# goroda/c3sc

Hardware: AMD Instinct MI355X
Metric: Bellman-sweep nodes/sec (7D car rank-10) (higher is better)
Workload: dtype f64

## Files before the change

c3sc_amd/csrc/kernel_fiber_pair.hpp:

```cpp
#pragma once
#include <utility>

#include "fold_lds.hpp"

#ifndef FPP_CGD
#define FPP_CGD 3
#endif
#ifndef FPP_PIPE2
#define FPP_PIPE2 1
#endif
#ifndef FPP_CG
#define FPP_CG 1
#endif
#ifndef FPP_NV
#define FPP_NV 4
#endif

#ifndef FPP_DIRECT_MAXD
#define FPP_DIRECT_MAXD 3
#endif
#ifndef FPP_EDGE_TABLES
#define FPP_EDGE_TABLES 1
#endif

namespace c3sc {

constexpr int FPP_THREADS = 128;

template <class Model, int RP>
__host__ __device__ constexpr bool fpp_direct() { return Model::D <= FPP_DIRECT_MAXD && RP <= 8; }

template <class Model, int RP>
__host__ __device__ constexpr bool fpp_edge_tables() { return FPP_EDGE_TABLES && !fpp_direct<Model, RP>() && Model::D >= 4; }

template <int RP>
__device__ __forceinline__ void load_row16(const double *__restrict__ p, double (&r)[RP])
{
    typedef double v2d __attribute__((ext_vector_type(2)));
#pragma unroll
    for (int i = 0; i < RP / 2; i++) {
        const v2d v = *reinterpret_cast<const v2d *>(p + 2 * i);
        r[2 * i] = v.x;
        r[2 * i + 1] = v.y;
    }
}

template <int RP, int NW, int FIRST, int COUNT, bool ROWVEC>
__device__ inline void apply_core_and(const double *G, double (&W)[NW][RP], double (&E)[RP])
{
    constexpr int N1 = COUNT >= FPP_NV - 1 ? FPP_NV - 1 : COUNT;
    double tmp[N1 + 1][RP];
#pragma unroll
    for (int a = 0; a < RP; a++) tmp[0][a] = E[a];
#pragma unroll
    for (int s = 0; s < N1; s++)
#pragma unroll
        for (int a = 0; a < RP; a++) tmp[s + 1][a] = W[FIRST + s][a];
    if constexpr (ROWVEC) vecmat_lds<RP, N1 + 1>(G, tmp);
    else matvec_lds<RP, N1 + 1>(G, tmp);
#pragma unroll
    for (int a = 0; a < RP; a++) E[a] = tmp[0][a];
#pragma unroll
    for (int s = 0; s < N1; s++)
#pragma unroll
        for (int a = 0; a < RP; a++) W[FIRST + s][a] = tmp[s + 1][a];
    apply_core<RP, NW, FIRST + N1, COUNT - N1, ROWVEC, FPP_NV>(G, W);
}

__device__ inline void pair_barrier()
{
    asm volatile("s_waitcnt lgkmcnt(0)\n\ts_barrier" ::: "memory");
}

template <int H>
__device__ inline void stage_core_image(double *sK, const double *img, int n_doubles)
{
    typedef __attribute__((address_space(3))) char lds_char;
    typedef __attribute__((address_space(3))) void lds_void;
    typedef const __attribute__((address_space(1))) void glb_void;
    const int pieces = (n_doubles + 1) >> 1;
    const int lane = threadIdx.x & 63;
    for (int base = H * 64; base < pieces; base += FPP_THREADS) {
        const int b = max(min(base, pieces - 64), 0);
        const int p = min(b + lane, pieces - 1);
        __builtin_amdgcn_global_load_lds((glb_void *)(img + 2 * p), (lds_void *)((lds_char *)sK + 16 * b), 16, 0, 0);
    }
    asm volatile("s_waitcnt vmcnt(0)" ::: "memory");
}

template <int K>
__host__ __device__ constexpr int pair_owner(int m) { return m < K ? ((K - 1 - m) & 1) : ((m - K) & 1); }

template <class Model, int K>
struct PairPark {
    static constexpr int D = Model::D, NTAB = Model::NTAB;
    static constexpr unsigned UM = Model::UDEP_MASK, UC = Model::UCONST_MASK, ALL = (1u << D) - 1u;
    __host__ __device__ static constexpr bool has_deps()
    {
        if constexpr (requires { Model::HAS_DEPS; }) return Model::HAS_DEPS;
        else return false;
    }
    __host__ __device__ static constexpr unsigned dep(int m)
    {
        if constexpr (has_deps()) return Model::dep_mask(m);
        else return ALL;
    }
    __host__ __device__ static constexpr unsigned cost_dep()
    {
        if constexpr (has_deps()) return Model::COST_DEP;
        else return ALL;
    }
    __host__ __device__ static constexpr unsigned constd()
    {
        unsigned c = 0;
        if (has_deps())
            for (int m = 0; m < D; m++)
                if (!((UM >> m) & 1u) && !((dep(m) >> K) & 1u)) c |= 1u << m;
        return c;
    }
    __host__ __device__ static constexpr unsigned need()
    {
        unsigned n = cost_dep();
        for (int m = 0; m < D; m++) {
            const bool ctl = (UM >> m) & 1u, cst = (constd() >> m) & 1u;
            if ((!ctl && !cst) || (ctl && !((UC >> m) & 1u))) n |= dep(m);
        }
        return n & ALL;
    }
    __host__ __device__ static constexpr bool need_x(int m) { return m != K && ((need() >> m) & 1u); }
    __host__ __device__ static constexpr bool need_t(int t) { return Model::tab_dim(t) != K && ((need() >> Model::tab_dim(t)) & 1u); }
    __host__ __device__ static constexpr int row_x(int m)
    {
        int r = 0;
        for (int q = 0; q < m; q++) r += need_x(q);
        return r;
    }
    __host__ __device__ static constexpr int nx() { return row_x(D); }
    __host__ __device__ static constexpr int row_t(int t)
    {
        int r = nx();
        for (int q = 0; q < t; q++) r += need_t(q);
        return r;
    }
    __host__ __device__ static constexpr int nt() { return row_t(NTAB) - nx(); }
    __host__ __device__ static constexpr unsigned merged() { return constd() & ~(1u << K); }
    __host__ __device__ static constexpr unsigned rates() { return constd() & (1u << K); }
    __host__ __device__ static constexpr int row_pm(int m)
    {
        int r = nx() + nt();
        for (int q = 0; q < m; q++) r += 2 * ((rates() >> q) & 1u);
        return r;
    }
    __host__ __device__ static constexpr int row_q() { return row_pm(D); }
    __host__ __device__ static constexpr int rows() { return row_q() + (merged() != 0u); }
};

struct FoldPlan {
    int lfirst, rfirst;
    bool ledge, redge;
    int staged;
    int products;
};
template <class Model, int K, bool TAB = false>
struct PairMap {
    typedef PairPark<Model, K> PK;
    static constexpr int D = Model::D, NIT = D + 2, UL = D, UR = D + 1;
    __host__ __device__ static constexpr bool ltab() { return TAB && K >= 2; }
    __host__ __device__ static constexpr bool rtab() { return TAB && K <= D - 3; }
    __host__ __device__ static constexpr bool mg(int m) { return (PK::merged() >> m) & 1u; }
    __host__ __device__ static constexpr int first_l()
    {
        for (int m = 0; m < K; m++)
            if (mg(m)) return m;
        return -1;
    }
    __host__ __device__ static constexpr int first_r()
    {
        for (int m = D - 1; m > K; m--)
            if (mg(m)) return m;
        return -1;
    }
    __host__ __device__ static constexpr bool valid(int it)
    {
        return it == UL ? first_l() >= 0 : (it == UR ? first_r() >= 0 : (it != K && !mg(it)));
    }
    __host__ __device__ static constexpr int count(int it) { return !valid(it) ? 0 : (it < D ? 2 : 1); }
    __host__ __device__ static constexpr int nvl()
    {
        int c = count(UL);
        for (int m = 0; m < K; m++) c += count(m);
        return c;
    }
    __host__ __device__ static constexpr int nvr()
    {
        int c = count(UR);
        for (int m = K + 1; m < D; m++) c += count(m);
        return c;
    }
    __host__ __device__ static constexpr int nv() { return nvl() + nvr(); }
    __host__ __device__ static constexpr int gslot(int it)
    {
        if (it == UL) return 0;
        if (it == UR) return nvl();
        int c = it < K ? count(UL) : nvl() + count(UR);
        for (int m = it < K ? 0 : K + 1; m < it; m++) c += count(m);
        return c;
    }
    __host__ __device__ static constexpr int cost(int it)
    {
        if (!valid(it)) return 0;
        constexpr int lf = ltab() ? 2 : 1, rf = rtab() ? D - 3 : D - 2;
        if (it == UL) {
            int c = K - 1 - first_l() - (ltab() && first_l() == 0);
            for (int m = lf; m < K; m++) c += 2 * mg(m);
            return c;
        }
        if (it == UR) {
            int c = first_r() - K - 1 - (rtab() && first_r() == D - 1);
            for (int m = K + 1; m <= rf; m++) c += 2 * mg(m);
            return c;
        }
        if (it < K) return (ltab() && it <= 1) ? 2 * (K - 2) : (it > 0 ? 2 : 0) + 2 * (K - 1 - it);
        return (rtab() && it >= D - 2) ? 2 * (D - 3 - K) : (it < D - 1 ? 2 : 0) + 2 * (it - K - 1);
    }
    __host__ __device__ static constexpr FoldPlan plan()
    {
        FoldPlan p{ltab() ? 2 : 1, rtab() ? D - 3 : D - 2, K > 0 && !TAB, K < D - 1 && !TAB, 0, 0};
        const int ls = K - p.lfirst > 0 ? K - p.lfirst : 0, rs = p.rfirst - K > 0 ? p.rfirst - K : 0;
        p.staged = ls + rs + p.ledge + p.redge;
        p.products = ls + rs;
        for (int it = 0; it < NIT; it++) p.products += cost(it);
        return p;
    }
    __host__ __device__ static constexpr int owner(int it)
    {
        if (PK::merged() == 0u) return pair_owner<K>(it);
        int load[2] = {0, 0}, own[NIT] = {};
        bool done[NIT] = {};
        for (int n = 0; n < NIT; n++) {
            int best = -1;
            for (int q = 0; q < NIT; q++)
                if (valid(q) && !done[q] && (best < 0 || cost(q) > cost(best))) best = q;
            if (best < 0) break;
            const int h = load[1] < load[0] ? 1 : 0;
            own[best] = h;
            load[h] += cost(best);
            done[best] = true;
        }
        return own[it];
    }
    __host__ __device__ static constexpr int created(int m)
    {
        if (m == K) return -1;
        if (!mg(m)) return m;
        return m < K ? (m == first_l() ? UL : -1) : (m == first_r() ? UR : -1);
    }
    template <int H>
    __host__ __device__ static constexpr int left_before(int m)
    {
        int c = 0;
        for (int q = 0; q < m && q < K; q++)
            if (created(q) >= 0 && owner(created(q)) == H) c += count(created(q));
        return c;
    }
    template <int H>
    __host__ __device__ static constexpr int right_after(int m)
    {
        int c = 0;
        for (int q = D - 1; q > m && q > K; q--)
            if (created(q) >= 0 && owner(created(q)) == H) c += count(created(q));
        return c;
    }
    template <int H>
    __host__ __device__ static constexpr int lslot(int it)
    {
        if (it == UL) return left_before<H>(first_l());
        if (it == UR) return left_before<H>(K) + right_after<H>(first_r());
        return it < K ? left_before<H>(it) : left_before<H>(K) + right_after<H>(it);
    }
};

template <class Model, int K>
struct PairPre {
    static constexpr unsigned MASK = PairPark<Model, K>::merged(), RATES = PairPark<Model, K>::rates();
    const double *PX;
    int lane;
    double pvc;
    __device__ inline double q() const { return PX[PairPark<Model, K>::row_q() * 64 + lane]; }
    __device__ inline double pv() const { return pvc; }
    __device__ inline double pm(int m) const { return PX[PairPark<Model, K>::row_pm(m) * 64 + lane]; }
    __device__ inline double pp(int m) const { return PX[(PairPark<Model, K>::row_pm(m) + 1) * 64 + lane]; }
};

#define FPP_STAMP(slot)                                                   \
    if (C3SC_STAMPS_ON && (A.dbg & 128)) {                                \
        const unsigned long long now__ = clock64();                       \
        seg[slot] += now__ - tlast;                                       \
        tlast = now__;                                                    \
    }

template <class Model, int RP, int K, int H, bool FORCED>
__device__ __attribute__((always_inline)) inline void fiber_pair_body(const KArgs &A, const double *__restrict__ ro,
                                                                     const int32_t *__restrict__ idx, double *__restrict__ outv,
                                                                     int32_t *__restrict__ uidx, int32_t *__restrict__ absorbed,
                                                                     double *sK, unsigned &st)
{
    constexpr int D = Model::D;
    constexpr int S = 2 * D + 1;
    constexpr int RH = RP / 2;
    typedef PairPark<Model, K> PK;
    constexpr bool ET = fpp_edge_tables<Model, RP>();
    typedef PairMap<Model, K, ET> PM;
    constexpr FoldPlan PL = PM::plan();
    constexpr int NV = PM::nv();
    constexpr int NVL = PM::nvl();
    constexpr int NOL = PM::template left_before<H>(K);
    constexpr int NOR = PM::template right_after<H>(K);
    constexpr int NOWN = (NOL + NOR) > 0 ? (NOL + NOR) : 1;
    constexpr int NP = NV + 1;
    constexpr bool DIRECT = fpp_direct<Model, RP>();
    static_assert(RP % 2 == 0, "rank-split kernel needs an even padded rank");
    const int lane = threadIdx.x & 63;
    const int N = A.N;
    const long ntiles = (A.F + 63) / 64;
    unsigned long long seg[12] = {0, 0, 0, 0, 0, 0, 0, 0, 0, 0, 0, 0}, tlast = clock64();
    CandLds<Model> cr;
    NodeLds<Model, K> nr;
    {
        CandRegs<Model> cr0;
        cr0.load(A, ro);
        NodeRegs<Model, K> nr0;
        nr0.load(A, ro);
        double *tb = sK + A.tbl_off;
        cr.fill(tb, cr0, A.ncand);
        nr.fill(tb + CandLds<Model>::doubles(A.ncand), nr0, N);
        pair_barrier();
    }

    for (long tile = blockIdx.x; tile < ntiles; tile += gridDim.x) {
        FPP_STAMP(7)
        const long f_raw = tile * 64 + lane;
        const bool live = f_raw < A.F;
        const long f = live ? f_raw : A.F - 1;

        int fi[D], nbm[D], nbp[D];
        bool fiber_abs = false;
        double x[D];
#pragma unroll
        for (int m = 0; m < D; m++) {
            fi[m] = (m == K) ? 0 : idx[f * D + m];
            const bool face = fixed_neighbors(fi[m], A.ngrid[m], A.bctype[m], nbm[m], nbp[m]);
            if (m != K) fiber_abs = fiber_abs || face;
            x[m] = ro[A.xg_off[m] + fi[m]];
        }

        const unsigned obs_fixed = obstacle_mask_fixed<D>(A, ro, x, K);
        double tv[Model::NTAB > 0 ? Model::NTAB : 1];
        table_values<Model>(A, ro, fi, tv);

        double rpm[D], rpp[D];
#pragma unroll
        for (int m = 0; m < D; m++) { rpm[m] = 0.0; rpp[m] = 0.0; }
        if constexpr (PK::constd() != 0) {
            typename Model::Node nd0;
            Model::prep(A.prm, x, tv, nd0);
            double u0[Model::DU], cf0[Model::NCF > 0 ? Model::NCF : 1], b0[D], s0[D];
#pragma unroll
            for (int i = 0; i < Model::DU; i++) u0[i] = cr.get_u(i, 0);
            cf0[0] = 0.0;
#pragma unroll
            for (int i = 0; i < Model::NCF; i++) cf0[i] = cr.get_cf(i, 0);
            Model::drift(A.prm, nd0, x, u0, cf0, b0);
            Model::sigma(A.prm, x, u0, s0);
#pragma unroll
            for (int m = 0; m < D; m++)
                if ((PK::constd() >> m) & 1u) upwind_rates(A.t[2 * m], A.t[2 * m + 1], b0[m], s0[m], rpm[m], rpp[m]);
        }

        double L[RP], R[RP], W[NOWN][RP];
#pragma unroll
        for (int a = 0; a < RP; a++) { L[a] = (a == 0) ? 1.0 : 0.0; R[a] = (a == 0) ? 1.0 : 0.0; }

        FPP_STAMP(0)
        if (!(C3SC_STAMPS_ON && (A.dbg & 1))) {
        if constexpr (K > 0) {
            constexpr bool OWN0 = PM::ltab() && (PM::mg(0) ? PM::owner(PM::UL) == H : PM::owner(0) == H);
            constexpr bool OWN1 = PM::ltab() && (PM::mg(1) ? PM::owner(PM::UL) == H : PM::owner(1) == H);
            double t0m[OWN0 ? RP : 1], t0p[OWN0 ? RP : 1], t1m[OWN1 ? RP : 1], t1p[OWN1 ? RP : 1];
            if constexpr (PM::ltab()) {
                const double *T = ro + pair_tabL_off(A, RP);
                const int n1 = A.ngrid[1];
                load_row16<RP>(T + ((long)fi[0] * n1 + fi[1]) * RP, L);
                if constexpr (OWN0) {
                    load_row16<RP>(T + ((long)nbm[0] * n1 + fi[1]) * RP, t0m);
                    load_row16<RP>(T + ((long)nbp[0] * n1 + fi[1]) * RP, t0p);
                }
                if constexpr (OWN1) {
                    load_row16<RP>(T + ((long)fi[0] * n1 + nbm[1]) * RP, t1m);
                    load_row16<RP>(T + ((long)fi[0] * n1 + nbp[1]) * RP, t1p);
                }
                __builtin_amdgcn_sched_barrier(0);
            }
            auto left_combine = [&]() __attribute__((always_inline)) {
                if constexpr (OWN0) {
#pragma unroll
                    for (int b = 0; b < RP; b++) {
                        if constexpr (PM::mg(0)) W[0][b] = fma(rpp[0], t0p[b], rpm[0] * t0m[b]);
                        else { W[0][b] = t0m[b]; W[1][b] = t0p[b]; }
                    }
                }
                if constexpr (OWN1) {
                    constexpr int before = PM::template left_before<H>(1);
#pragma unroll
                    for (int b = 0; b < RP; b++) {
                        if constexpr (PM::mg(1)) {
                            constexpr int su = PM::template lslot<H>(PM::UL);
                            const double nw = fma(rpp[1], t1p[b], rpm[1] * t1m[b]);
                            W[su][b] = (1 == PM::first_l()) ? nw : W[su][b] + nw;
                        } else { W[before][b] = t1m[b]; W[before + 1][b] = t1p[b]; }
                    }
                }
            };
            if constexpr (PM::ltab() && K == PL.lfirst) left_combine();
            if constexpr (!PM::ltab()) {
                constexpr bool GLB = DIRECT || !PL.ledge;
                constexpr int str = GLB ? RP : fpl_lds_stride(RP);
                const double *src = sK;
                FPP_STAMP(1)
                if constexpr (GLB) src = ro + A.core_off[0];
                else {
                    pair_barrier();
                    stage_core_image<H>(sK, A.img_base + A.pair_img_off[0], A.ngrid[0] * str);
                    pair_barrier();
                }
                FPP_STAMP(7)
#pragma unroll
                for (int b = 0; b < RP; b++) {
                    L[b] = src[fi[0] * str + b];
                    if constexpr (PM::mg(0)) {
                        if constexpr (PM::owner(PM::UL) == H) W[0][b] = fma(rpp[0], src[nbp[0] * str + b], rpm[0] * src[nbm[0] * str + b]);
                    } else if constexpr (PM::owner(0) == H) {
                        W[0][b] = src[nbm[0] * str + b];
                        W[1][b] = src[nbp[0] * str + b];
                    }
                }
            }
            auto left_step = [&](auto mc) __attribute__((always_inline)) {
                constexpr int m = decltype(mc)::value;
                constexpr int str = DIRECT ? RP * RP : fpl_lds_stride(RP * RP);
                constexpr int before = PM::template left_before<H>(m);
                constexpr bool PAIR = !PM::mg(m) && PM::owner(m) == H, ACC = PM::mg(m) && PM::owner(PM::UL) == H;
                double nw[RP];
                const double *src = sK;
                FPP_STAMP(1)
                if constexpr (DIRECT) src = ro + A.core_off[m];
                else {
                    pair_barrier();
                    stage_core_image<H>(sK, A.img_base + A.pair_img_off[m], A.ngrid[m] * str);
                    pair_barrier();
                }
                if constexpr (PM::ltab() && m == PL.lfirst) left_combine();
                FPP_STAMP(7)
                const double *G = src + fi[m] * str;
                if constexpr (PAIR || ACC) {
                    double t0[1][RP], t1[1][RP];
#pragma unroll
                    for (int a = 0; a < RP; a++) { t0[0][a] = L[a]; t1[0][a] = L[a]; }
                    if constexpr (DIRECT) {
                        apply_glb<RP, 1, true>(src + nbm[m] * str, t0);
                        apply_glb<RP, 1, true>(src + nbp[m] * str, t1);
                    } else {
                        vecmat_lds<RP, 1>(src + nbm[m] * str, t0);
                        vecmat_lds<RP, 1>(src + nbp[m] * str, t1);
                    }
#pragma unroll
                    for (int a = 0; a < RP; a++) {
                        if constexpr (PAIR) { W[before][a] = t0[0][a]; W[before + 1][a] = t1[0][a]; }
                        else nw[a] = fma(rpp[m], t1[0][a], rpm[m] * t0[0][a]);
                    }
                }
                if constexpr (DIRECT) {
                    double tl[1][RP];
#pragma unroll
                    for (int a = 0; a < RP; a++) tl[0][a] = L[a];
                    apply_glb<RP, 1, true>(G, tl);
#pragma unroll
                    for (int a = 0; a < RP; a++) L[a] = tl[0][a];
                    apply_range_glb<RP, NOWN, 0, before, true>(G, W);
                } else
                    apply_core_and<RP, NOWN, 0, before, true>(G, W, L);
                if constexpr (ACC) {
                    constexpr int su = PM::template lslot<H>(PM::UL);
#pragma unroll
                    for (int a = 0; a < RP; a++) W[su][a] = (m == PM::first_l()) ? nw[a] : W[su][a] + nw[a];
                }
            };
            [&]<int... Ms>(std::integer_sequence<int, Ms...>) { (left_step(std::integral_constant<int, Ms + PL.lfirst>{}), ...); }
            (std::make_integer_sequence<int, (K > PL.lfirst ? K - PL.lfirst : 0)>{});
        }

        if constexpr (K < D - 1) {
            constexpr bool OWN0 = PM::rtab() && (PM::mg(D - 1) ? PM::owner(PM::UR) == H : PM::owner(D - 1) == H);
            constexpr bool OWN1 = PM::rtab() && (PM::mg(D - 2) ? PM::owner(PM::UR) == H : PM::owner(D - 2) == H);
            double t0m[OWN0 ? RP : 1], t0p[OWN0 ? RP : 1], t1m[OWN1 ? RP : 1], t1p[OWN1 ? RP : 1];
            if constexpr (PM::rtab()) {
                const double *T = ro + pair_tabR_off(A, RP);
                const int n1 = A.ngrid[D - 1];
                load_row16<RP>(T + ((long)fi[D - 2] * n1 + fi[D - 1]) * RP, R);
                if constexpr (OWN0) {
                    load_row16<RP>(T + ((long)fi[D - 2] * n1 + nbm[D - 1]) * RP, t0m);
                    load_row16<RP>(T + ((long)fi[D - 2] * n1 + nbp[D - 1]) * RP, t0p);
                }
                if constexpr (OWN1) {
                    load_row16<RP>(T + ((long)nbm[D - 2] * n1 + fi[D - 1]) * RP, t1m);
                    load_row16<RP>(T + ((long)nbp[D - 2] * n1 + fi[D - 1]) * RP, t1p);
                }
                __builtin_amdgcn_sched_barrier(0);
            }
            auto right_combine = [&]() __attribute__((always_inline)) {
                if constexpr (OWN0) {
#pragma unroll
                    for (int a = 0; a < RP; a++) {
                        if constexpr (PM::mg(D - 1)) W[NOL][a] = fma(rpp[D - 1], t0p[a], rpm[D - 1] * t0m[a]);
                        else { W[NOL][a] = t0m[a]; W[NOL + 1][a] = t0p[a]; }
                    }
                }
                if constexpr (OWN1) {
                    constexpr int after = PM::template right_after<H>(D - 2);
#pragma unroll
                    for (int a = 0; a < RP; a++) {
                        if constexpr (PM::mg(D - 2)) {
                            constexpr int su = PM::template lslot<H>(PM::UR);
                            const double nw = fma(rpp[D - 2], t1p[a], rpm[D - 2] * t1m[a]);
                            W[su][a] = (D - 2 == PM::first_r()) ? nw : W[su][a] + nw;
                        } else { W[NOL + after][a] = t1m[a]; W[NOL + after + 1][a] = t1p[a]; }
                    }
                }
            };
            if constexpr (PM::rtab() && K == PL.rfirst) right_combine();
            if constexpr (!PM::rtab()) {
                constexpr bool GLB = DIRECT || !PL.redge;
                constexpr int str = GLB ? RP : fpl_lds_stride(RP);
                const double *src = sK;
                FPP_STAMP(1)
                if constexpr (GLB) src = ro + A.core_off[D - 1];
                else {
                    pair_barrier();
                    stage_core_image<H>(sK, A.img_base + A.pair_img_off[D - 1], A.ngrid[D - 1] * str);
                    pair_barrier();
                }
                FPP_STAMP(7)
#pragma unroll
                for (int a = 0; a < RP; a++) {
                    R[a] = src[fi[D - 1] * str + a];
                    if constexpr (PM::mg(D - 1)) {
                        if constexpr (PM::owner(PM::UR) == H)
                            W[NOL][a] = fma(rpp[D - 1], src[nbp[D - 1] * str + a], rpm[D - 1] * src[nbm[D - 1] * str + a]);
                    } else if constexpr (PM::owner(D - 1) == H) {
                        W[NOL][a] = src[nbm[D - 1] * str + a];
                        W[NOL + 1][a] = src[nbp[D - 1] * str + a];
                    }
                }
            }
            auto right_step = [&](auto mc) __attribute__((always_inline)) {
                constexpr int m = decltype(mc)::value;
                constexpr int str = DIRECT ? RP * RP : fpl_lds_stride(RP * RP);
                constexpr int after = PM::template right_after<H>(m);
                constexpr bool PAIR = !PM::mg(m) && PM::owner(m) == H, ACC = PM::mg(m) && PM::owner(PM::UR) == H;
                double nw[RP];
                const double *src = sK;
                FPP_STAMP(1)
                if constexpr (DIRECT) src = ro + A.core_off[m];
                else {
                    pair_barrier();
                    stage_core_image<H>(sK, A.img_base + A.pair_img_off[m], A.ngrid[m] * str);
                    pair_barrier();
                }
                if constexpr (PM::rtab() && m == PL.rfirst) right_combine();
                FPP_STAMP(7)
                const double *G = src + fi[m] * str;
                if constexpr (PAIR || ACC) {
                    double t0[1][RP], t1[1][RP];
#pragma unroll
                    for (int a = 0; a < RP; a++) { t0[0][a] = R[a]; t1[0][a] = R[a]; }
                    if constexpr (DIRECT) {
                        apply_glb<RP, 1, false>(src + nbm[m] * str, t0);
                        apply_glb<RP, 1, false>(src + nbp[m] * str, t1);
                    } else {
                        matvec_lds<RP, 1>(src + nbm[m] * str, t0);
                        matvec_lds<RP, 1>(src + nbp[m] * str, t1);
                    }
#pragma unroll
                    for (int a = 0; a < RP; a++) {
                        if constexpr (PAIR) { W[NOL + after][a] = t0[0][a]; W[NOL + after + 1][a] = t1[0][a]; }
                        else nw[a] = fma(rpp[m], t1[0][a], rpm[m] * t0[0][a]);
                    }
                }
                if constexpr (DIRECT) {
                    double tr[1][RP];
#pragma unroll
                    for (int a = 0; a < RP; a++) tr[0][a] = R[a];
                    apply_glb<RP, 1, false>(G, tr);
#pragma unroll
                    for (int a = 0; a < RP; a++) R[a] = tr[0][a];
                    apply_range_glb<RP, NOWN, NOL, after, false>(G, W);
                } else
                    apply_core_and<RP, NOWN, NOL, after, false>(G, W, R);
                if constexpr (ACC) {
                    constexpr int su = PM::template lslot<H>(PM::UR);
#pragma unroll
                    for (int a = 0; a < RP; a++) W[su][a] = (m == PM::first_r()) ? nw[a] : W[su][a] + nw[a];
                }
            };
            [&]<int... Ms>(std::integer_sequence<int, Ms...>) { (right_step(std::integral_constant<int, PL.rfirst - Ms>{}), ...); }
            (std::make_integer_sequence<int, (PL.rfirst - K > 0 ? PL.rfirst - K : 0)>{});
        }

        }
        FPP_STAMP(1)
        double Wh[NV][RH];
        {
            double *X = sK;
            pair_barrier();
            auto put_get_own = [&](auto ic) __attribute__((always_inline)) {
                constexpr int it = decltype(ic)::value;
                if constexpr (PM::valid(it) && PM::owner(it) == H) {
                    constexpr int slot = PM::template lslot<H>(it);
#pragma unroll
                    for (int s = 0; s < PM::count(it); s++) {
                        const int g = PM::gslot(it) + s;
#pragma unroll
                        for (int i = 0; i < RH; i++) {
                            X[(g * RH + i) * 64 + lane] = W[slot + s][(1 - H) * RH + i];
                            Wh[g][i] = W[slot + s][H * RH + i];
                        }
                    }
                }
            };
            [&]<int... Ms>(std::integer_sequence<int, Ms...>) { (put_get_own(std::integral_constant<int, Ms>{}), ...); }
            (std::make_integer_sequence<int, PM::NIT>{});
            pair_barrier();
            auto get_other = [&](auto ic) __attribute__((always_inline)) {
                constexpr int it = decltype(ic)::value;
                if constexpr (PM::valid(it) && PM::owner(it) != H) {
#pragma unroll
                    for (int s = 0; s < PM::count(it); s++) {
                        const int g = PM::gslot(it) + s;
#pragma unroll
                        for (int i = 0; i < RH; i++) Wh[g][i] = X[(g * RH + i) * 64 + lane];
                    }
                }
            };
            [&]<int... Ms>(std::integer_sequence<int, Ms...>) { (get_other(std::integral_constant<int, Ms>{}), ...); }
            (std::make_integer_sequence<int, PM::NIT>{});
            pair_barrier();
        }
        double *sL = sK, *sR = sK + RP * 64;
        {
#pragma unroll
            for (int a = 0; a < RP; a++) {
                if constexpr (H == 0) sL[a * 64 + lane] = L[a];
                else sR[a * 64 + lane] = R[a];
            }
            if constexpr (H == 0) {
                static_assert(PK::rows() <= NP, "parking rows exceed the reserved block");
                double *PXw = sK + (2 * RP + 2 * (NP + 1) + NP) * 64;
#pragma unroll
                for (int m = 0; m < D; m++)
                    if (PK::need_x(m)) PXw[PK::row_x(m) * 64 + lane] = x[m];
#pragma unroll
                for (int t = 0; t < Model::NTAB; t++)
                    if (PK::need_t(t)) PXw[PK::row_t(t) * 64 + lane] = tv[t];
#pragma unroll
                for (int m = 0; m < D; m++)
                    if ((PK::rates() >> m) & 1u) {
                        PXw[PK::row_pm(m) * 64 + lane] = rpm[m];
                        PXw[(PK::row_pm(m) + 1) * 64 + lane] = rpp[m];
                    }
                if constexpr (PK::merged() != 0u) {
                    double qc = 0.0;
#pragma unroll
                    for (int m = 0; m < D; m++)
                        if (PM::mg(m)) { qc += rpm[m]; qc += rpp[m]; }
                    PXw[PK::row_q() * 64 + lane] = qc;
                }
            }
            pair_barrier();
        }
        FPP_STAMP(2)

        const int bck = A.bctype[K];
        const double *Gk = ro + A.core_off[K];
        auto partials = [&](int j, auto &&sink) __attribute__((always_inline)) -> double {
            double pv;
            if constexpr (K == 0) {
                double ah[RH];
#pragma unroll
                for (int i = 0; i < RH; i++) ah[i] = Gk[(size_t)j * RP + H * RH + i];
                double v = 0.0;
#pragma unroll
                for (int i = 0; i < RH; i++) v = fma(ah[i], sR[(H * RH + i) * 64 + lane], v);
                pv = v;
#pragma unroll
                for (int g = 0; g < NV; g++) sink(g, dot_reg<RH>(ah, Wh[g]));
            } else if constexpr (K == D - 1) {
                double ch[RH];
#pragma unroll
                for (int i = 0; i < RH; i++) ch[i] = Gk[(size_t)j * RP + H * RH + i];
                double v = 0.0;
#pragma unroll
                for (int i = 0; i < RH; i++) v = fma(sL[(H * RH + i) * 64 + lane], ch[i], v);
                pv = v;
#pragma unroll
                for (int g = 0; g < NV; g++) sink(g, dot_reg<RH>(Wh[g], ch));
            } else {
                const double *GC0 = Gk + (size_t)j * RP * RP;
                const double *GC = GC0 + (size_t)H * RH * RP;
                double ch[RH], ah[RH];
#pragma unroll
                for (int i = 0; i < RH; i++) { ch[i] = 0.0; ah[i] = 0.0; }
#pragma unroll
                for (int b = 0; b < RP; b++) {
                    const double rb = sR[b * 64 + lane];
#pragma unroll
                    for (int i = 0; i < RH; i++) ch[i] = fma(GC0[H * RH + i + b * RP], rb, ch[i]);
                }
#pragma unroll
                for (int a = 0; a < RP; a++) {
                    const double la = sL[a * 64 + lane];
#pragma unroll
                    for (int i = 0; i < RH; i++) ah[i] = fma(la, GC[a + i * RP], ah[i]);
                }
                double v = 0.0;
#pragma unroll
                for (int i = 0; i < RH; i++) v = fma(sL[(H * RH + i) * 64 + lane], ch[i], v);
                pv = v;
#pragma unroll
                for (int g = 0; g < NVL; g++) sink(g, dot_reg<RH>(Wh[g], ch));
#pragma unroll
                for (int g = NVL; g < NV; g++) sink(g, dot_reg<RH>(ah, Wh[g]));
            }
            sink(NV, pv);
            return pv;
        };
        auto to_lds = [&](double *dst) __attribute__((always_inline)) {
            return [dst, lane](int g, double v) __attribute__((always_inline)) { dst[g * 64 + lane] = v; };
        };
        auto ca_part = [&](int j, double (&ch)[RH], double (&ah)[RH], auto &&filler) __attribute__((always_inline)) {
            const double *GC0 = Gk + (size_t)j * RP * RP;
            const double *GC = GC0 + (size_t)H * RH * RP;
#pragma unroll
            for (int i = 0; i < RH; i++) { ch[i] = 0.0; ah[i] = 0.0; }
            constexpr int BH = (RP + 1) / 2;
            double vec[RP];
#pragma unroll
            for (int b = 0; b < RP; b++) vec[b] = sR[b * 64 + lane];
#pragma unroll
            for (int b0 = 0; b0 < RP; b0 += BH) {
                double g[BH][RH];
#pragma unroll
                for (int b = 0; b < BH; b++)
#pragma unroll
                    for (int i = 0; i < RH; i++) g[b][i] = (b0 + b < RP) ? GC0[H * RH + i + (b0 + b) * RP] : 0.0;
                __builtin_amdgcn_sched_barrier(0);
                filler(b0 / BH);
                __builtin_amdgcn_sched_barrier(0);
#pragma unroll
                for (int b = 0; b < BH; b++)
#pragma unroll
                    for (int i = 0; i < RH; i++) asm volatile("" : "+s"(g[b][i]));
#pragma unroll
                for (int b = 0; b < BH; b++) {
                    if (b0 + b < RP) {
                        const double rb = vec[b0 + b];
#pragma unroll
                        for (int i = 0; i < RH; i++) ch[i] = fma(g[b][i], rb, ch[i]);
                    }
                }
            }
#pragma unroll
            for (int a = 0; a < RP; a++) vec[a] = sL[a * 64 + lane];
#pragma unroll
            for (int a0 = 0; a0 < RP; a0 += BH) {
                double g[RH][BH];
#pragma unroll
                for (int i = 0; i < RH; i++)
#pragma unroll
                    for (int a = 0; a < BH; a++) g[i][a] = (a0 + a < RP) ? GC[a0 + a + i * RP] : 0.0;
                __builtin_amdgcn_sched_barrier(0);
                filler(2 + a0 / BH);
                __builtin_amdgcn_sched_barrier(0);
#pragma unroll
                for (int i = 0; i < RH; i++)
#pragma unroll
                    for (int a = 0; a < BH; a++) asm volatile("" : "+s"(g[i][a]));
#pragma unroll
                for (int a = 0; a < BH; a++) {
                    if (a0 + a < RP) {
                        const double la = vec[a0 + a];
#pragma unroll
                        for (int i = 0; i < RH; i++) ah[i] = fma(la, g[i][a], ah[i]);
                    }
                }
            }
        };
        auto dots_quarter = [&](int q, const double (&ch)[RH], const double (&ah)[RH], auto &&sink) __attribute__((always_inline)) {
#pragma unroll
            for (int g = 0; g < NV; g++)
                if (g * 4 / NV == q) sink(g, (g < NVL) ? dot_reg<RH>(Wh[g], ch) : dot_reg<RH>(ah, Wh[g]));
        };
        auto dots_part = [&](const double (&ch)[RH], const double (&ah)[RH], auto &&sink) __attribute__((always_inline)) -> double {
            double v = 0.0;
#pragma unroll
            for (int i = 0; i < RH; i++) v = fma(sL[(H * RH + i) * 64 + lane], ch[i], v);
#pragma unroll
            for (int g = 0; g < NVL; g++) sink(g, dot_reg<RH>(Wh[g], ch));
#pragma unroll
            for (int g = NVL; g < NV; g++) sink(g, dot_reg<RH>(ah, Wh[g]));
            sink(NV, v);
            return v;
        };
        double *B0 = sK + 2 * RP * 64;
        double *B1 = B0 + (NP + 1) * 64;
        double *B2 = B1 + (NP + 1) * 64;
        double *PX = B2 + NP * 64;

        auto finalize = [&](int jn, const double (&Vt)[NP], double vlo, double vhi) __attribute__((always_inline)) {
            double V[S];
#pragma unroll
            for (int m = 0; m < D; m++) {
                if (m == K) { V[2 * m] = vlo; V[2 * m + 1] = vhi; }
                else if (PM::mg(m)) { V[2 * m] = 0.0; V[2 * m + 1] = 0.0; }
                else { V[2 * m] = Vt[PM::gslot(m)]; V[2 * m + 1] = Vt[PM::gslot(m) + 1]; }
            }
            V[2 * D] = Vt[NV];
            double pvc = 0.0;
            if constexpr (PM::valid(PM::UL)) pvc += Vt[PM::gslot(PM::UL)];
            if constexpr (PM::valid(PM::UR)) pvc += Vt[PM::gslot(PM::UR)];
            double x[D], tv[Model::NTAB > 0 ? Model::NTAB : 1];
            tv[0] = 0.0;
#pragma unroll
            for (int m = 0; m < D; m++)
                x[m] = (m == K) ? nr.x_at(jn) : (PairPark<Model, K>::need_x(m) ? PX[PairPark<Model, K>::row_x(m) * 64 + lane] : 0.0);
#pragma unroll
            for (int t = 0; t < Model::NTAB; t++)
                tv[t] = (Model::tab_dim(t) == K) ? nr.tab_at(t, jn)
                                                 : (PairPark<Model, K>::need_t(t) ? PX[PairPark<Model, K>::row_t(t) * 64 + lane] : 0.0);
            int ab = (obs_fixed & nr.mask_at(jn)) ? -1 : 0;
            if (fiber_abs) ab = 1;
            int lo, hi;
            ab = vary_neighbors(jn, N, bck, ab, lo, hi, A.cends);
            int ui;
            FPP_STAMP(8)
            int fu = -1;
            if constexpr (FORCED) fu = A.forced[(size_t)f * N + jn];
            const PairPre<Model, K> pre{PX, lane, pvc};
            const double val = node_backup<Model, FPP_CG, FPP_CGD, CandLds<Model>, true, PairPre<Model, K>>(A, ro, x, tv, cr, V, ab, ui, st, FORCED, fu, pre);
            FPP_STAMP(9)
            outv[(size_t)f * N + jn] = val;
            if (uidx) uidx[(size_t)f * N + jn] = ui;
            if (absorbed) absorbed[(size_t)f * N + jn] = ab;
        };

        double vwrap = 0.0;
        if (bck == C3SC_PERIODIC) {
            const double pv = partials(N - 2, [](int, double) __attribute__((always_inline)) {});
            if constexpr (H == 0) B0[NP * 64 + lane] = pv;
            else B1[NP * 64 + lane] = pv;
            pair_barrier();
            vwrap = pv + (H == 0 ? B1[NP * 64 + lane] : B0[NP * 64 + lane]);
            pair_barrier();
        }
        double vone = 0.0;
        double v_m2 = 0.0, v_m1 = 0.0;
        double Vd[NP];
#pragma unroll
        for (int g = 0; g < NP; g++) Vd[g] = 0.0;

        const int T = N / 2 + 1;
        for (int t = 0; t < T; t++) {
            const int j0 = 2 * t, j1 = 2 * t + 1;
            const bool has0 = j0 < N, has1 = j1 < N;
            double pv0 = 0.0, pv1 = 0.0;
            double Pown[NP];
#pragma unroll
            for (int g = 0; g < NP; g++) Pown[g] = 0.0;
            auto own_sink = [&](int g, double v) __attribute__((always_inline)) { Pown[g] = v; };
            if constexpr (K > 0 && K < D - 1 && FPP_PIPE2) {
                if (has0 && has1) {
                    double chA[RH], ahA[RH], chB[RH], ahB[RH];
                    auto nofill = [](int) __attribute__((always_inline)) {};
                    auto value_of = [&](const double (&ch)[RH]) __attribute__((always_inline)) -> double {
                        double v = 0.0;
#pragma unroll
                        for (int i = 0; i < RH; i++) v = fma(sL[(H * RH + i) * 64 + lane], ch[i], v);
                        return v;
                    };
                    if constexpr (H == 0) {
                        auto sinkA = to_lds(B0);
                        ca_part(j1, chA, ahA, nofill);
                        ca_part(j0, chB, ahB, [&](int q) __attribute__((always_inline)) { dots_quarter(q, chA, ahA, sinkA); });
                        pv1 = value_of(chA);
                        sinkA(NV, pv1);
                        pv0 = dots_part(chB, ahB, own_sink);
                        B0[NP * 64 + lane] = pv0;
                    } else {
                        auto sinkA = to_lds(B1);
                        ca_part(j0, chA, ahA, nofill);
                        ca_part(j1, chB, ahB, [&](int q) __attribute__((always_inline)) { dots_quarter(q, chA, ahA, sinkA); });
                        pv0 = value_of(chA);
                        sinkA(NV, pv0);
                        pv1 = dots_part(chB, ahB, to_lds(B2));
                        B1[NP * 64 + lane] = pv1;
                    }
                } else if (has0) {
                    if constexpr (H == 0) { pv0 = partials(j0, own_sink); B0[NP * 64 + lane] = pv0; }
                    else pv0 = partials(j0, to_lds(B1));
                }
            } else if constexpr (H == 0) {
                if (has1) pv1 = partials(j1, to_lds(B0));
                if (has0) {
                    pv0 = partials(j0, own_sink);
                    B0[NP * 64 + lane] = pv0;
                }
            } else {
                if (has0) pv0 = partials(j0, to_lds(B1));
                if (has1) {
                    pv1 = partials(j1, to_lds(B2));
                    B1[NP * 64 + lane] = pv1;
                }
            }
            FPP_STAMP(3)
            pair_barrier();
            FPP_STAMP(4)
            double v0 = 0.0, v1 = 0.0;
            if constexpr (H == 0) {
                if (has1) v1 = pv1 + B1[NP * 64 + lane];
                if (has0) {
                    double P0[NP];
#pragma unroll
                    for (int g = 0; g < NP; g++) P0[g] = Pown[g] + B1[g * 64 + lane];
                    v0 = P0[NV];
                    double vlo, vhi;
                    dimk_values(j0, N, bck, v_m1, v0, v1, vwrap, (j0 == 0 ? v1 : vone), vlo, vhi);
                    finalize(j0, P0, vlo, vhi);
                }
            } else {
                if (has0) v0 = pv0 + B0[NP * 64 + lane];
                if (t >= 1) {
                    const int jn = j0 - 1;
                    double vlo, vhi;
                    dimk_values(jn, N, bck, v_m2, Vd[NV], v0, vwrap, (jn == 1 ? Vd[NV] : vone), vlo, vhi);
                    finalize(jn, Vd, vlo, vhi);
                }
                if (has1) {
#pragma unroll
                    for (int g = 0; g < NP; g++) Vd[g] = B0[g * 64 + lane] + B2[g * 64 + lane];
                    v1 = Vd[NV];
                }
            }
            if (t == 0) vone = v1;
            v_m2 = v0;
            v_m1 = v1;
            FPP_STAMP(5)
            pair_barrier();
            FPP_STAMP(6)
        }
    }
    if (C3SC_STAMPS_ON && (A.dbg & 128) && lane == 0) {
        const size_t w = ((size_t)blockIdx.x * 2 + H) * 12;
        if (w < 65536 * 8)
            for (int i = 0; i < 12; i++) A.dbgbuf[w + i] = seg[i];
    }
}

#ifndef FPP_WPS_LOW
#define FPP_WPS_LOW 4
#endif
#ifndef FPP_WPS_HIGH
#define FPP_WPS_HIGH 2
#endif
template <class Model, int RP>
__host__ __device__ constexpr int fpp_waves_per_simd() { return (fpp_direct<Model, RP>() && RP <= 6) ? FPP_WPS_LOW : (FPP_WPS_HIGH); }

template <class Model, int RP, int K, bool FORCED>
__global__ void __launch_bounds__(FPP_THREADS, (fpp_waves_per_simd<Model, RP>()))
    k_fiber_pair(const KArgs A, const double *__restrict__ ro, const int32_t *__restrict__ idx, double *__restrict__ outv,
                 int32_t *__restrict__ uidx, int32_t *__restrict__ absorbed)
{
    extern __shared__ double sKp[];
    unsigned st = 0;
    const int h = __builtin_amdgcn_readfirstlane(threadIdx.x >> 6);
    if (h == 0) fiber_pair_body<Model, RP, K, 0, FORCED>(A, ro, idx, outv, uidx, absorbed, sKp, st);
    else fiber_pair_body<Model, RP, K, 1, FORCED>(A, ro, idx, outv, uidx, absorbed, sKp, st);
    if (st) atomicOr(A.status, st);
}

}
```

c3sc_amd/csrc/launch_fpp.hpp:

```cpp
#pragma once
#include "kernel_fiber_pair.hpp"
#include "registry.hpp"

namespace c3sc {

template <class Model, int RP, int K, bool FORCED>
hipError_t launch_fpp_impl(const KArgs &A, const LaunchIO &io)
{
    constexpr int D = Model::D;
    constexpr int NV = PairMap<Model, K>::nv(), NP = NV + 1, RH = RP / 2;
    if (A.ncand > 64) return hipErrorNotSupported;
    size_t doubles = (size_t)NV * RH * 64;
    const size_t exch = (size_t)(2 * RP + (NP + 1) * 2 + 2 * NP) * 64;
    if (exch > doubles) doubles = exch;
    for (int m = 0; m < D; m++) {
        if (m == K || fpp_direct<Model, RP>()) continue;
        const int elems = (m == 0 || m == D - 1) ? RP : RP * RP;
        const size_t need = ((size_t)A.ngrid[m] * fpl_lds_stride(elems) + 1) & ~(size_t)1;
        if (need > doubles) doubles = need;
    }
    KArgs B = A;
    B.tbl_off = (int)doubles;
    doubles += (size_t)CandLds<Model>::doubles(A.ncand) + (size_t)NodeLds<Model, K>::doubles(A.N);
    const size_t shmem = doubles * sizeof(double);
    auto kern = k_fiber_pair<Model, RP, K, FORCED>;
    static LaunchCache cache;
    int blocks_per_cu = 1, num_cu = 256;
    hipError_t e = cache.prepare((const void *)kern, FPP_THREADS, shmem, blocks_per_cu, num_cu);
    if (e != hipSuccess) return e;
    const long ntiles = (A.F + 63) / 64;
    const long cap = (long)num_cu * blocks_per_cu;
    int grid = (int)(ntiles < cap ? ntiles : cap);
    if (ntiles >= 8 * cap && ntiles < 0x7fffffffL) grid = (int)ntiles;
    if (grid < 1) grid = 1;
    hipLaunchKernelGGL(kern, dim3(grid), dim3(FPP_THREADS), shmem, io.stream, B, io.ro, io.idx, io.out, io.uidx, io.absorbed);
    return hipGetLastError();
}

template <class Model, int RP, int K>
hipError_t launch_fpp(const KArgs &A, const LaunchIO &io)
{
    return A.forced ? launch_fpp_impl<Model, RP, K, true>(A, io) : launch_fpp_impl<Model, RP, K, false>(A, io);
}

#define C3SC_REG_FPP1(MODEL_ID, RP, K, ...)                                                                   \
    static Registrar C3SC_CAT(reg_fpp_, __COUNTER__)(KernelEntry{                                             \
        MODEL_ID, __VA_ARGS__::D, RP, 0, C3SC_VARIANT_FIBER_PAIR, 128, K, &launch_fpp<__VA_ARGS__, RP, K>, \
        "k_fiber_pair<" #__VA_ARGS__ "," #RP ",K=" #K ">"});

}
```

Before: 29.86 billion.

## Split fiber-pair node work by node parity instead of by rank half

Adds a node-split mode where each wave of the pair keeps full-rank W vectors (exchanged via LDS in two halves) and computes the complete stencil for alternating nodes, instead of each wave computing half-rank partials that are summed through LDS every node. This removes per-node partial-sum exchange and one barrier per step, at the cost of more VGPRs (full NV×RP registers) and duplicated stencil reads. It is gated by a VGPR budget and opts out for rank<10 and the 7D rank-10 K=4 case. LDS sizing is refactored into a helper with static asserts.

Result: faster. 31.40 billion (median of 6 runs) (+5.2%).

```diff
diff --git a/c3sc_amd/csrc/kernel_fiber_pair.hpp b/c3sc_amd/csrc/kernel_fiber_pair.hpp
--- a/c3sc_amd/csrc/kernel_fiber_pair.hpp
+++ b/c3sc_amd/csrc/kernel_fiber_pair.hpp
@@ -21,6 +21,13 @@
 #endif
 #ifndef FPP_EDGE_TABLES
 #define FPP_EDGE_TABLES 1
+#endif
+
+#ifndef FPP_NODE_SPLIT
+#define FPP_NODE_SPLIT 1
+#endif
+#ifndef FPP_NODE_SPLIT_VGPRS
+#define FPP_NODE_SPLIT_VGPRS 140
 #endif
 
 namespace c3sc {
@@ -279,6 +286,16 @@
         return it < K ? left_before<H>(it) : left_before<H>(K) + right_after<H>(it);
     }
 };
+
+__host__ __device__ constexpr bool fpp_node_split_optout(int d, int rp, int k) { return rp < 10 || (d == 7 && rp == 10 && k == 4); }
+template <class Model, int RP, int K>
+__host__ __device__ constexpr bool fpp_node_split()
+{
+    if constexpr (!FPP_NODE_SPLIT || fpp_direct<Model, RP>()) return false;
+    else
+        return PairPark<Model, K>::merged() != 0u && PairMap<Model, K>::nv() * RP * 2 <= FPP_NODE_SPLIT_VGPRS &&
+               !fpp_node_split_optout(Model::D, RP, K);
+}
 
 template <class Model, int K>
 struct PairPre {
@@ -618,8 +635,49 @@
 
         }
         FPP_STAMP(1)
-        double Wh[NV][RH];
-        {
+        constexpr bool NS = fpp_node_split<Model, RP, K>();
+        double Wh[NS ? 1 : NV][RH];
+        double Wf[NS ? NV : 1][RP];
+        if constexpr (NS) {
+            double *X = sK;
+            auto put_get_own = [&](auto ic, auto pc) __attribute__((always_inline)) {
+                constexpr int it = decltype(ic)::value, P = decltype(pc)::value;
+                if constexpr (PM::valid(it) && PM::owner(it) == H) {
+                    constexpr int slot = PM::template lslot<H>(it);
+#pragma unroll
+                    for (int s = 0; s < PM::count(it); s++) {
+                        const int g = PM::gslot(it) + s;
+#pragma unroll
+                        for (int i = 0; i < RH; i++) {
+                            X[(g * RH + i) * 64 + lane] = W[slot + s][P * RH + i];
+                            Wf[g][P * RH + i] = W[slot + s][P * RH + i];
+                        }
+                    }
+                }
+            };
+            auto get_other = [&](auto ic, auto pc) __attribute__((always_inline)) {
+                constexpr int it = decltype(ic)::value, P = decltype(pc)::value;
+                if constexpr (PM::valid(it) && PM::owner(it) != H) {
+#pragma unroll
+                    for (int s = 0; s < PM::count(it); s++) {
+                        const int g = PM::gslot(it) + s;
+#pragma unroll
+                        for (int i = 0; i < RH; i++) Wf[g][P * RH + i] = X[(g * RH + i) * 64 + lane];
+                    }
+                }
+            };
+            auto half = [&](auto pc) __attribute__((always_inline)) {
+                pair_barrier();
+                [&]<int... Ms>(std::integer_sequence<int, Ms...>) { (put_get_own(std::integral_constant<int, Ms>{}, pc), ...); }
+                (std::make_integer_sequence<int, PM::NIT>{});
+                pair_barrier();
+                [&]<int... Ms>(std::integer_sequence<int, Ms...>) { (get_other(std::integral_constant<int, Ms>{}, pc), ...); }
+                (std::make_integer_sequence<int, PM::NIT>{});
+            };
+            half(std::integral_constant<int, 0>{});
+            half(std::integral_constant<int, 1>{});
+            pair_barrier();
+        } else {
             double *X = sK;
             pair_barrier();
             auto put_get_own = [&](auto ic) __attribute__((always_inline)) {
@@ -862,6 +920,128 @@
             if (absorbed) absorbed[(size_t)f * N + jn] = ab;
         };
 
+        if constexpr (NS) {
+        auto stencil = [&](int j, double (&Vt)[NP]) __attribute__((always_inline)) {
+            double v = 0.0;
+            if constexpr (K == 0) {
+                double a[RP];
+#pragma unroll
+                for (int i = 0; i < RP; i++) a[i] = Gk[(size_t)j * RP + i];
+#pragma unroll
+                for (int i = 0; i < RP; i++) v = fma(a[i], sR[i * 64 + lane], v);
+#pragma unroll
+                for (int g = 0; g < NV; g++) Vt[g] = dot_reg<RP>(a, Wf[g]);
+            } else if constexpr (K == D - 1) {
+                double c[RP];
+#pragma unroll
+                for (int i = 0; i < RP; i++) c[i] = Gk[(size_t)j * RP + i];
+#pragma unroll
+                for (int i = 0; i < RP; i++) v = fma(sL[i * 64 + lane], c[i], v);
+#pragma unroll
+                for (int g = 0; g < NV; g++) Vt[g] = dot_reg<RP>(Wf[g], c);
+            } else {
+                const double *G0 = Gk + (size_t)j * RP * RP;
+                constexpr int NE = RP * RP, NB = (NE + 3) / 4;
+                double c[RP], a[RP], lv[RP];
+#pragma unroll
+                for (int i = 0; i < RP; i++) lv[i] = sL[i * 64 + lane];
+#pragma unroll
+                for (int i = 0; i < RP; i++) { c[i] = 0.0; a[i] = 0.0; }
+#pragma unroll
+                for (int b0 = 0; b0 < NE; b0 += NB) {
+                    double g[NB];
+#pragma unroll
+                    for (int e = 0; e < NB; e++) g[e] = (b0 + e < NE) ? G0[b0 + e] : 0.0;
+                    double rv[RP];
+#pragma unroll
+                    for (int p = 0; p < RP; p++) rv[p] = (p >= b0 / RP && p * RP < b0 + NB) ? sR[p * 64 + lane] : 0.0;
+                    __builtin_amdgcn_sched_barrier(0);
+#pragma unroll
+                    for (int e = 0; e < NB; e++) asm volatile("" : "+s"(g[e]));
+#pragma unroll
+                    for (int e = 0; e < NB; e++) {
+                        if (b0 + e < NE) {
+                            const int p = (b0 + e) / RP, q = (b0 + e) % RP;
+                            c[q] = fma(g[e], rv[p], c[q]);
+                            a[p] = fma(lv[q], g[e], a[p]);
+                        }
+                    }
+#pragma unroll
+                    for (int i = 0; i < RP; i++) asm volatile("" : "+v"(c[i]), "+v"(a[i]));
+                }
+#pragma unroll
+                for (int i = 0; i < RP; i++) v = fma(sL[i * 64 + lane], c[i], v);
+#pragma unroll
+                for (int g = 0; g < NVL; g++) Vt[g] = dot_reg<RP>(Wf[g], c);
+#pragma unroll
+                for (int g = NVL; g < NV; g++) Vt[g] = dot_reg<RP>(a, Wf[g]);
+            }
+            Vt[NV] = v;
+        };
+        double *VX = B0;
+        double vwrap = 0.0;
+        if (bck == C3SC_PERIODIC) {
+            double Vw[NP];
+            stencil(N - 2, Vw);
+            vwrap = Vw[NV];
+        }
+        double vone = 0.0;
+        double v_m2 = 0.0, v_m1 = 0.0;
+        double Vd[NP];
+#pragma unroll
+        for (int g = 0; g < NP; g++) Vd[g] = 0.0;
+        const int T = N / 2 + 1;
+        for (int t = 0; t < T; t++) {
+            const int j0 = 2 * t, j1 = 2 * t + 1;
+            const bool has0 = j0 < N, has1 = j1 < N;
+            double *vx = VX + (t & 1) * 64;
+            double v0 = 0.0, v1 = 0.0;
+            double Pn[NP];
+#pragma unroll
+            for (int g = 0; g < NP; g++) Pn[g] = 0.0;
+            if constexpr (H == 0) {
+                if (has0) {
+                    stencil(j0, Pn);
+                    v0 = Pn[NV];
+                    vx[lane] = v0;
+                }
+                FPP_STAMP(3)
+                pair_barrier();
+                FPP_STAMP(4)
+                if (has1) v1 = vx[2 * 64 + lane];
+                if (has0) {
+                    double vlo, vhi;
+                    dimk_values(j0, N, bck, v_m1, v0, v1, vwrap, (j0 == 0 ? v1 : vone), vlo, vhi);
+                    finalize(j0, Pn, vlo, vhi);
+                }
+            } else {
+                if (has1) {
+                    stencil(j1, Pn);
+                    v1 = Pn[NV];
+                    vx[2 * 64 + lane] = v1;
+                }
+                FPP_STAMP(3)
+                pair_barrier();
+                FPP_STAMP(4)
+                if (has0) v0 = vx[lane];
+                if (t >= 1) {
+                    const int jn = j0 - 1;
+                    double vlo, vhi;
+                    dimk_values(jn, N, bck, v_m2, Vd[NV], v0, vwrap, (jn == 1 ? Vd[NV] : vone), vlo, vhi);
+                    finalize(jn, Vd, vlo, vhi);
+                }
+                if (has1) {
+#pragma unroll
+                    for (int g = 0; g < NP; g++) Vd[g] = Pn[g];
+                }
+            }
+            if (t == 0) vone = v1;
+            v_m2 = v0;
+            v_m1 = v1;
+            FPP_STAMP(5)
+        }
+        pair_barrier();
+        } else {
         double vwrap = 0.0;
         if (bck == C3SC_PERIODIC) {
             const double pv = partials(N - 2, [](int, double) __attribute__((always_inline)) {});
@@ -966,6 +1146,7 @@
             pair_barrier();
             FPP_STAMP(6)
         }
+        }
     }
     if (C3SC_STAMPS_ON && (A.dbg & 128) && lane == 0) {
         const size_t w = ((size_t)blockIdx.x * 2 + H) * 12;
diff --git a/c3sc_amd/csrc/launch_fpp.hpp b/c3sc_amd/csrc/launch_fpp.hpp
--- a/c3sc_amd/csrc/launch_fpp.hpp
+++ b/c3sc_amd/csrc/launch_fpp.hpp
@@ -4,15 +4,25 @@
 
 namespace c3sc {
 
+template <class Model, int RP, int K>
+__host__ __device__ constexpr size_t fpp_tile_doubles(bool node_split)
+{
+    constexpr int NV = PairMap<Model, K>::nv(), NP = NV + 1, RH = RP / 2;
+    const size_t swap = (size_t)NV * RH * 64;
+    const size_t parked = (size_t)(2 * RP + (NP + 1) * 2 + NP) * 64;
+    const size_t rows = node_split ? parked + (size_t)PairPark<Model, K>::rows() * 64 : parked + (size_t)NP * 64;
+    return swap > rows ? swap : rows;
+}
+
 template <class Model, int RP, int K, bool FORCED>
 hipError_t launch_fpp_impl(const KArgs &A, const LaunchIO &io)
 {
     constexpr int D = Model::D;
-    constexpr int NV = PairMap<Model, K>::nv(), NP = NV + 1, RH = RP / 2;
     if (A.ncand > 64) return hipErrorNotSupported;
-    size_t doubles = (size_t)NV * RH * 64;
-    const size_t exch = (size_t)(2 * RP + (NP + 1) * 2 + 2 * NP) * 64;
-    if (exch > doubles) doubles = exch;
+    constexpr bool NS = fpp_node_split<Model, RP, K>();
+    static_assert(fpp_tile_doubles<Model, RP, K>(NS) <= fpp_tile_doubles<Model, RP, K>(false), "the node split must not need more LDS than the rank split");
+    static_assert(!NS || 4 * fpp_tile_doubles<Model, RP, K>(NS) * sizeof(double) <= 160 * 1024, "four node-split workgroups per CU must fit the LDS");
+    size_t doubles = fpp_tile_doubles<Model, RP, K>(false);
     for (int m = 0; m < D; m++) {
         if (m == K || fpp_direct<Model, RP>()) continue;
         const int elems = (m == 0 || m == D - 1) ? RP : RP * RP;
```
